# InnaBoby/Speech-Enhancement-via-Hybrid-Vision-Transformer-Project

Measured on AMD Instinct MI355X. Metric: spectrogram-frames/sec/GPU (fwd+bwd) on 256x256 mag-spec, batch 32; 1/2/4/8 GPU, higher is better.
Workload: dtype bf16; 1 GPU; HybridViT default (enc 64/128/256, 6x8-head d512 ViT, dec 256/128/64/1) train step: fwd + CombinedLoss + bwd + clip + AdamW; global_batch=32, seq_len=256, parallelism=dp1

## Files before the change

include/hvit.h:

```cpp
#ifndef HVIT_H_
#define HVIT_H_

#ifdef __cplusplus
extern "C" {
#endif

enum { HVIT_F32 = 0, HVIT_BF16 = 1 };
enum { HVIT_OK = 0, HVIT_ERR_ARG = 1, HVIT_ERR_LAUNCH = 2 };
enum {
  HVIT_ACT_NONE = 0,
  HVIT_ACT_GELU_DUAL = 1,
  HVIT_ACT_TANH = 2,
  HVIT_ACT_GELU_BWD = 3,
  HVIT_ACT_GELU_DUAL_D = 4,
  HVIT_ACT_MUL_AUX = 5,
  HVIT_ACT_RELU = 6,
  HVIT_ACT_GELU = 7,
  HVIT_ACT_RELU_POOL2 = 8,
  HVIT_ACT_GELU_DUAL_DK = 9
};
enum { HVIT_ACC_ZEROED = 1,
       HVIT_ACC_DEFER = 2 };

typedef struct {
// ... 25 lines not shown
  int rowadd_rows;
  float* colsum;
  hvit_slab_sum_t side;
} hvit_epilogue_t;

typedef struct {
  const void* src1;
  int C1;
  const void* src2;
  int C2;
  int N, Hs, Ws, U;
  int KS, stride, pad;
  int Cout;
} hvit_conv_geom_t;

const char* hvit_last_error(void);
const char* hvit_version(void);

int hvit_linear_fwd(int dt, const void* x, const void* w, const float* bias, int M, int N, int K, void* y,
                    int y_dt, const hvit_epilogue_t* epi, void* stream);
int hvit_linear_dgrad(int dt, const void* dy, const void* w, int M, int N, int K, void* dx, int dx_dt,
                      const hvit_epilogue_t* epi, void* stream);
long long hvit_wgrad_workspace(int M, int N, int K);
long long hvit_wgrad_tickets(int M, int N, int K);
int hvit_linear_wgrad_tk(int dt, const void* dy, const void* x, int M, int N, int K, float* dw, float* db, float* ws,
                         long long ws_elems, unsigned* tickets, long long tickets_elems, int flags, void* stream);
enum {
  HVIT_TUNE_RING = 0,
  HVIT_TUNE_C1_MFMA = 1,
  HVIT_TUNE_ATTN_BWD = 4,
  HVIT_TUNE_FP8_FWD = 5,
  HVIT_TUNE_WGRAD_GROUP = 7,
  HVIT_TUNE_CONV_HALO = 9,
  HVIT_TUNE_CONV_HALO_COUNT = 10
};
int hvit_gemm_tune(int what, int value);
int hvit_conv_halo_off(int H, int W, int C, int rows, int hy, int hx, int chunk);
int hvit_linear_wgrad(int dt, const void* dy, const void* x, int M, int N, int K, float* dw, float* db,
                      float* ws, long long ws_elems, void* stream);
int hvit_linear_wgrad_defer(int dt, const void* dy, const void* x, int M, int N, int K, float* dw, float* ws,
                            long long ws_elems, const hvit_slab_sum_t* side, hvit_slab_sum_t* job, void* stream);
int hvit_linear_wgrad_bias_defer(int dt, const void* dy, const void* x, int M, int N, int K, float* dw, float* db,
                                 float* ws, long long ws_elems, const hvit_slab_sum_t* side, hvit_slab_sum_t* job,
                                 void* stream);
int hvit_sum_slabs_strided(const float* ws, int splits, long long stride, long long n, float* out, void* stream);

typedef struct {
  const void* dy;
  int ldy;
  const void* x;
  int ldx;
  float* dw;
  int n_out, k_in;
  int patch, img_h, img_w, img_c;
} hvit_wgrad_prob_t;
int hvit_linear_wgrad_group_ok(int dt, int M, int n_out, int k_in);
int hvit_linear_wgrad_group_patch_ok(int dt, int M, int n_out, int patch, int img_h, int img_w, int img_c);
long long hvit_linear_wgrad_group_ws(void);
long long hvit_linear_wgrad_group_tickets(void);
int hvit_linear_wgrad_group(int dt, int M, const hvit_wgrad_prob_t* probs, int nprobs, float* ws, long long ws_elems,
                            unsigned* tickets, long long n_tickets, void* stream);

int hvit_conv_bn_tile_rows(const hvit_conv_geom_t* g);
int hvit_conv_fwd(int dt, const hvit_conv_geom_t* g, const void* w_packed, const float* bias, void* y, int y_dt,
                  float* bn_partials, const hvit_epilogue_t* epi, void* stream);
int hvit_conv_dgrad(int dt, const hvit_conv_geom_t* g, const void* dy, const void* w_packed, void* dx, int dx_dt,
                    void* stream);
long long hvit_conv_wgrad_workspace(const hvit_conv_geom_t* g);
int hvit_conv_wgrad(int dt, const hvit_conv_geom_t* g, const void* dy, float* dw_packed, float* ws,
                    long long ws_elems, void* stream);
int hvit_conv_wgrad_torch(int dt, const hvit_conv_geom_t* g, const void* dy, float* dw, float* dw_packed, float* ws,
                          long long ws_elems, void* stream);
int hvit_conv_weight_pack(const float* w, int Cout, int Cin, int KS, int mode, void* out, int out_dt,
                          void* stream);
int hvit_conv_weight_unpack(const float* dw_packed, int Cout, int Cin, int KS, float* dw, void* stream);
int hvit_bn_fold(const float* w, int Cout, int Cin, int KS, const float* mean, const float* invstd,
                 const float* gamma, const float* beta, void* w_packed, int w_dt, float* bias, void* stream);

int hvit_mhsa_fwd(int dt, const void* qkv, int B, int N, int H, int hd, float scale,
                  const hvit_dropout_t* dropout, void* o, float* lse, float* probs, void* stream);
int hvit_mhsa_bwd(int dt, const void* qkv, const void* o, const void* dout, const float* lse, int B, int N, int H,
                  int hd, float scale, const hvit_dropout_t* dropout, void* dqkv, float* delta_ws, void* stream);
long long hvit_mhsa_keep_bits_elems(int B, int N, int H);
int hvit_mhsa_keep_bits_used(int dt, int N, int hd);
int hvit_mhsa_fwd_kb(int dt, const void* qkv, int B, int N, int H, int hd, float scale, const hvit_dropout_t* dropout,
                     void* o, float* lse, unsigned* keep_bits, void* stream);
int hvit_mhsa_bwd_kb(int dt, const void* qkv, const void* o, const void* dout, const float* lse, int B, int N, int H,
                     int hd, float scale, const hvit_dropout_t* dropout, const unsigned* keep_bits, void* dqkv,
                     float* delta_ws, void* stream);
long long hvit_mhsa_bias_rows(int dt, int B, int N, int H, int hd);
int hvit_mhsa_bwd_db(int dt, const void* qkv, const void* o, const void* dout, const float* lse, int B, int N, int H,
                     int hd, float scale, const hvit_dropout_t* dropout, const unsigned* keep_bits, void* dqkv,
                     float* delta_ws, float* dbias_rows, void* stream);
int hvit_mhsa_fwd_fp8(const void* qkv, int B, int N, int H, int hd, float scale, const hvit_dropout_t* dropout,
                      void* o, float* lse, void* stream);
int hvit_mhsa_fwd_fp8_kb(const void* qkv, int B, int N, int H, int hd, float scale, const hvit_dropout_t* dropout,
                         void* o, float* lse, unsigned* keep_bits, void* stream);

int hvit_layernorm_fwd(const float* x, const float* gamma, const float* beta, int M, int D, float eps, void* y,
                       int y_dt, float* mean, float* rstd, void* stream);
long long hvit_layernorm_bwd_ws_elems(int M, int D);
long long hvit_layernorm_bwd_drop_ws_elems(int M, int D);
int hvit_layernorm_bwd_drop(const void* dy, int dy_dt, const float* x, const float* mean, const float* rstd,
                            const float* gamma, int M, int D, const float* resid, float* dx, float* acc3,
                            const hvit_dropout_t* dropout, const float* rowscale, int rows_per_sample, void* g_out,
                            int g_dt, float* ws, long long ws_elems, int flags, void* stream);
int hvit_layernorm_bwd(const void* dy, int dy_dt, const float* x, const float* mean, const float* rstd,
                       const float* gamma, int M, int D, const float* resid, float* dx, float* dgamma,
                       float* dbeta, float* ws, long long ws_elems, int flags, void* stream);

long long hvit_bn_act_bwd_sums_elems(int C);
int hvit_bn_finalize(float* partials, int ntiles, int tile_rows, long long M, int C, float* mean,
                     float* invstd, float* running_mean, float* running_var, long long* num_batches_tracked,
                     float momentum, float eps, void* stream);
int hvit_bn_eval_prep(const float* running_mean, const float* running_var, int C, float eps, float* mean,
                      float* invstd, void* stream);
int hvit_bn_act_fwd(int dt, const void* z, int N, int H, int W, int C, const float* mean, const float* invstd,
                    const float* gamma, const float* beta, const hvit_dropout_t* dropout2d, int pool, void* y,
                    int y_dt, void* stream);
int hvit_bn_act_bwd(int dt, const void* z, int N, int H, int W, int C, const float* mean, const float* invstd,
                    const float* gamma, const float* beta, const hvit_dropout_t* dropout2d, int pool,
                    const void* dy, int dy_dt, int training, void* dz, int dz_dt, float* sums, int flags,
                    void* stream);

int hvit_c1block_stats(int dt, const hvit_conv_geom_t* g, const void* w_packed, float* bn_partials, void* stream);
int hvit_c1block_fwd(int dt, const hvit_conv_geom_t* g, const void* w_packed, const float* mean,
// ... 107 lines not shown
```

speech-enhancement-via-hybrid-vision-transformer-project_amd/_lib.py:

```python

from __future__ import annotations

import ctypes as C
import os
import threading

import torch

F32, BF16 = 0, 1
ACT_NONE, ACT_GELU_DUAL, ACT_TANH, ACT_GELU_BWD, ACT_GELU_DUAL_D, ACT_MUL_AUX, ACT_RELU, ACT_GELU, ACT_RELU_POOL2 = (
    0, 1, 2, 3, 4, 5, 6, 7, 8)
ACT_GELU_DUAL_DK = 9
ACC_ZEROED = 1
ACC_DEFER = 2
TUNE_RING, TUNE_C1_MFMA, TUNE_ATTN_BWD, TUNE_FP8_FWD, TUNE_WGRAD_GROUP, TUNE_CONV_HALO, TUNE_CONV_HALO_COUNT = (
    0, 1, 4, 5, 7, 9, 10)

_HERE = os.path.dirname(os.path.abspath(__file__))
LIB_PATH = os.path.join(_HERE, os.environ.get("HVIT_LIB", "libhvit.so"))

vp = C.c_void_p
i32 = C.c_int
i64 = C.c_longlong
f32 = C.c_float
f64 = C.c_double


class Dropout(C.Structure):
    _fields_ = [("p", C.c_float), ("seed", C.c_ulonglong), ("site", C.c_uint), ("seed_ptr", C.c_void_p)]


class SlabSum(C.Structure):
    _fields_ = [("src", vp), ("dst", vp), ("n", i64), ("stride", i64), ("splits", i32)]


class WgradProb(C.Structure):
    _fields_ = [("dy", vp), ("ldy", i32), ("x", vp), ("ldx", i32), ("dw", vp), ("n_out", i32), ("k_in", i32),
                ("patch", i32), ("img_h", i32), ("img_w", i32), ("img_c", i32)]


class Epilogue(C.Structure):
    _fields_ = [
        ("act", i32), ("out2", vp), ("out2_dt", i32), ("aux", vp), ("aux_dt", i32),
        ("dropout", Dropout), ("resid", vp), ("rowscale", vp), ("rows_per_sample", i32),
        ("rowadd", vp), ("rowadd_rows", i32), ("colsum", vp), ("side", SlabSum),
    ]


class ConvGeom(C.Structure):
# ... 40 lines not shown
    "hvit_last_error": ([], C.c_char_p),
    "hvit_version": ([], C.c_char_p),
    "hvit_linear_fwd": ([i32, vp, vp, vp, i32, i32, i32, vp, i32, P(Epilogue), vp], i32),
    "hvit_linear_dgrad": ([i32, vp, vp, i32, i32, i32, vp, i32, P(Epilogue), vp], i32),
    "hvit_wgrad_workspace": ([i32, i32, i32], i64),
    "hvit_linear_wgrad": ([i32, vp, vp, i32, i32, i32, vp, vp, vp, i64, vp], i32),
    "hvit_wgrad_tickets": ([i32, i32, i32], i64),
    "hvit_linear_wgrad_defer": ([i32, vp, vp, i32, i32, i32, vp, vp, i64, P(SlabSum), P(SlabSum), vp], i32),
    "hvit_linear_wgrad_bias_defer": ([i32, vp, vp, i32, i32, i32, vp, vp, vp, i64, P(SlabSum), P(SlabSum), vp],
                                     i32),
    "hvit_mhsa_bias_rows": ([i32, i32, i32, i32, i32], i64),
    "hvit_sum_slabs_strided": ([vp, i32, i64, i64, vp, vp], i32),
    "hvit_linear_wgrad_group_ok": ([i32, i32, i32, i32], i32),
    "hvit_linear_wgrad_group_patch_ok": ([i32, i32, i32, i32, i32, i32, i32], i32),
    "hvit_linear_wgrad_group_ws": ([], i64),
    "hvit_linear_wgrad_group_tickets": ([], i64),
    "hvit_linear_wgrad_group": ([i32, i32, P(WgradProb), i32, vp, i64, vp, i64, vp], i32),
    "hvit_linear_wgrad_tk": ([i32, vp, vp, i32, i32, i32, vp, vp, vp, i64, vp, i64, i32, vp], i32),
    "hvit_conv_fwd": ([i32, P(ConvGeom), vp, vp, vp, i32, vp, P(Epilogue), vp], i32),
    "hvit_conv_dgrad": ([i32, P(ConvGeom), vp, vp, vp, i32, vp], i32),
    "hvit_conv_wgrad_workspace": ([P(ConvGeom)], i64),
    "hvit_conv_wgrad": ([i32, P(ConvGeom), vp, vp, vp, i64, vp], i32),
    "hvit_conv_wgrad_torch": ([i32, P(ConvGeom), vp, vp, vp, vp, i64, vp], i32),
    "hvit_conv_weight_pack": ([vp, i32, i32, i32, i32, vp, i32, vp], i32),
    "hvit_conv_weight_unpack": ([vp, i32, i32, i32, vp, vp], i32),
    "hvit_bn_fold": ([vp, i32, i32, i32, vp, vp, vp, vp, vp, i32, vp, vp], i32),
    "hvit_mhsa_fwd": ([i32, vp, i32, i32, i32, i32, f32, P(Dropout), vp, vp, vp, vp], i32),
    "hvit_mhsa_fwd_fp8": ([vp, i32, i32, i32, i32, f32, P(Dropout), vp, vp, vp], i32),
    "hvit_mhsa_fwd_fp8_kb": ([vp, i32, i32, i32, i32, f32, P(Dropout), vp, vp, vp, vp], i32),
    "hvit_mhsa_bwd": ([i32, vp, vp, vp, vp, i32, i32, i32, i32, f32, P(Dropout), vp, vp, vp], i32),
    "hvit_mhsa_keep_bits_elems": ([i32, i32, i32], i64),
    "hvit_mhsa_keep_bits_used": ([i32, i32, i32], i32),
    "hvit_mhsa_fwd_kb": ([i32, vp, i32, i32, i32, i32, f32, P(Dropout), vp, vp, vp, vp], i32),
    "hvit_mhsa_bwd_kb": ([i32, vp, vp, vp, vp, i32, i32, i32, i32, f32, P(Dropout), vp, vp, vp, vp], i32),
    "hvit_mhsa_bwd_db": ([i32, vp, vp, vp, vp, i32, i32, i32, i32, f32, P(Dropout), vp, vp, vp, vp, vp], i32),
    "hvit_layernorm_fwd": ([vp, vp, vp, i32, i32, f32, vp, i32, vp, vp, vp], i32),
    "hvit_layernorm_bwd_ws_elems": ([i32, i32], i64),
    "hvit_layernorm_bwd_drop_ws_elems": ([i32, i32], i64),
    "hvit_layernorm_bwd_drop": ([vp, i32, vp, vp, vp, vp, i32, i32, vp, vp, vp, P(Dropout), vp, i32, vp, i32, vp,
                                 i64, i32, vp], i32),
    "hvit_layernorm_bwd": ([vp, i32, vp, vp, vp, vp, i32, i32, vp, vp, vp, vp, vp, i64, i32, vp], i32),
    "hvit_bn_finalize": ([vp, i32, i32, i64, i32, vp, vp, vp, vp, vp, f32, f32, vp], i32),
    "hvit_bn_eval_prep": ([vp, vp, i32, f32, vp, vp, vp], i32),
    "hvit_bn_act_fwd": ([i32, vp, i32, i32, i32, i32, vp, vp, vp, vp, P(Dropout), i32, vp, i32, vp], i32),
    "hvit_bn_act_bwd": ([i32, vp, i32, i32, i32, i32, vp, vp, vp, vp, P(Dropout), i32, vp, i32, i32, vp,
                         i32, vp, i32, vp], i32),
    "hvit_bn_act_bwd_sums_elems": ([i32], i64),
    "hvit_c1block_stats": ([i32, P(ConvGeom), vp, vp, vp], i32),
    "hvit_c1block_fwd": ([i32, P(ConvGeom), vp, vp, vp, vp, vp, P(Dropout), i32, vp, i32, vp], i32),
    "hvit_c1block_bwd_ws": ([P(ConvGeom), i32], i64),
    "hvit_c1block_bwd": ([i32, P(ConvGeom), vp, vp, vp, vp, vp, P(Dropout), i32, vp, i32, i32, vp, i32, vp, vp,
                          i64, vp], i32),
    "hvit_bilinear_fwd":([vp, i32, i32, i32, i32, i32, i32, i32, vp, i32, vp], i32),
    "hvit_bilinear_bwd": ([vp, i32, i32, i32, i32, i32, i32, i32, vp, i32, i32, vp], i32),
    "hvit_upsample_split_bwd": ([vp, i32, i32, i32, i32, i32, i32, i32, vp, i32, vp, i32, vp], i32),
    "hvit_cast": ([vp, i32, vp, i32, i64, vp], i32),
    "hvit_dropout_scale": ([vp, i32, i64, i32, P(Dropout), vp, i32, vp, i32, vp, vp, i64, vp], i32),
    "hvit_dropout_colsum_ws_elems": ([i32], i64),
    "hvit_tanh_bwd": ([vp, i32, vp, i64, vp, i32, vp], i32),
    "hvit_reduce_rows": ([vp, i32, i64, i64, i64, i32, vp, vp], i32),
    "hvit_sum_slabs": ([vp, i32, i64, vp, vp], i32),
    "hvit_droppath_scale": ([i32, P(Dropout), vp, vp], i32),
    "hvit_droppath_scales": ([i32, i32, P(Dropout), vp, vp], i32),
    "hvit_weight_prep": ([i32, P(WPrepItem), vp], i32),
    "hvit_conv_bn_tile_rows": ([P(ConvGeom)], i32),
    "hvit_loss_ws_elems": ([i32, i64], i64),
# ... 102 lines not shown
```

speech-enhancement-via-hybrid-vision-transformer-project_amd/csrc/attention.hip:

```cpp
#include <algorithm>
#include <cstdlib>

#include "attention_tile.h"
#include "common.h"

namespace hvit {

constexpr int AT_THREADS = 256;
constexpr int AT_TILE = 64;

template <typename T>
__device__ __forceinline__ f32x4 mma_step(u32x4 a, u32x4 b, f32x4 c) {
  if constexpr (sizeof(T) == 2) {
    return __builtin_amdgcn_mfma_f32_16x16x32_bf16(__builtin_bit_cast(s16x8, a),
                                                   __builtin_bit_cast(s16x8, b), c, 0, 0, 0);
  } else {
    f32x4 va = __builtin_bit_cast(f32x4, a), vb = __builtin_bit_cast(f32x4, b);
    c = __builtin_amdgcn_mfma_f32_16x16x4f32(va[0], vb[0], c, 0, 0, 0);
    c = __builtin_amdgcn_mfma_f32_16x16x4f32(va[1], vb[1], c, 0, 0, 0);
    c = __builtin_amdgcn_mfma_f32_16x16x4f32(va[2], vb[2], c, 0, 0, 0);
    c = __builtin_amdgcn_mfma_f32_16x16x4f32(va[3], vb[3], c, 0, 0, 0);
    return c;
  }
}
// ... 387 lines not shown
#pragma unroll
      for (int r = 0; r < 4; ++r)
        *(T*)(Pw + (4 * fq + r) * GK::PITCH + (16 * j + frow) * sizeof(T)) = Elem<T>::from_f(s[j][r]);
    lds_fence();
#pragma unroll
    for (int st = 0; st < GK::STEPS; ++st) {
      u32x4 pa = frag<GK>(Pw, frow, st, fq);
#pragma unroll
      for (int t = 0; t < NT; ++t) dk[t] = mma_step<T>(pa, frag<GK>(Qt, 16 * t + frow, st, fq), dk[t]);
    }
    lds_fence();
  }
#pragma unroll
  for (int r = 0; r < 4; ++r) {
    int kj = key0 + 4 * fq + r;
    if (kj >= N) continue;
    T* row = dqkv + ((long)b * N + kj) * pitch + h * HD;
#pragma unroll
    for (int t = 0; t < NT; ++t) {
      row[D + 16 * t + frow] = Elem<T>::from_f(dk[t][r] * scale);
      row[2 * D + 16 * t + frow] = Elem<T>::from_f(dv[t][r]);
    }
  }
}

constexpr int V2_KMAX = 512;

template <int WAVES, int KMAX, bool FULL = false>
__global__ __launch_bounds__(WAVES * 64) void mhsa_fwd_v2(const bf16_t* __restrict__ qkv, bf16_t* __restrict__ o,
                                                         float* __restrict__ lse, int N, int H, float scale,
                                                         uint32_t thr, float dscale, DSeed seed_,
                                                         uint32_t site, uint32_t* __restrict__ kbits) {
  const unsigned long long seed = seed_;
  constexpr int CH = 256;
  __shared__ __attribute__((aligned(16))) char smem[2 * KMAX * V2_ROWB];
  char* Ks = smem;
  char* Vs = smem + KMAX * V2_ROWB;
  const int D = H * 64;
  const long pitch = 3L * D;
  const int h = blockIdx.y, b = blockIdx.z;
  const int lane = threadIdx.x & 63, w = threadIdx.x >> 6;
  const int frow = lane & 15, fq = lane >> 4;
  const V2Lane LN(lane);
  const bf16_t* base = qkv + (long)b * N * pitch + h * 64;
  const int NK32 = (N + 31) & ~31;
  const int q = blockIdx.x * WAVES * 16 + w * 16 + frow;
  const bool qin = FULL || q < N;
  u32x4 qf[2];
#pragma unroll
  for (int s2 = 0; s2 < 2; ++s2)
    qf[s2] = qin ? *(const u32x4*)(base + (long)q * pitch + 32 * s2 + 8 * fq) : (u32x4){0u, 0u, 0u, 0u};
  v2_stage_glds<WAVES>(Ks, base + D, pitch, N, NK32);
  v2_stage_glds<WAVES>(Vs, base + 2 * D, pitch, N, NK32);
  __syncthreads();
  const float c2 = scale * 1.4426950408889634f;
  const uint64_t bh = (uint64_t)b * H + h;
  const uint64_t BHN = (uint64_t)gridDim.z * H * N;
  const uint32_t rk = rng_key(seed, site);
  const uint64_t qrow = (bh * N + (qin ? q : 0)) * (uint64_t)N;
  const uint32_t hq = (uint32_t)(qrow >> 1) + 2u * (uint32_t)fq;
  f32x4 ot[4];
#pragma unroll
  for (int t = 0; t < 4; ++t) ot[t] = (f32x4){0.f, 0.f, 0.f, 0.f};
  float mxc = -INFINITY, sum = 0.f;
  auto chunk = [&](auto c0c) {
    constexpr int c0 = decltype(c0c)::value;
    const int nkt = FULL ? CH / 16 : (min(N - c0, CH) + 15) >> 4;
    const char* Kc = Ks + c0 * V2_ROWB;
    const char* Vc = Vs + c0 * V2_ROWB;
    f32x4 st[CH / 16];
    float mx = -INFINITY;
#pragma unroll
    for (int j = 0; j < CH / 16; ++j) {
      if (j < nkt) {
        f32x4 a = {0.f, 0.f, 0.f, 0.f};
        a = v2_mma32(v2_fragj(Kc, LN, j, 0), qf[0], a);
        a = v2_mma32(v2_fragj(Kc, LN, j, 1), qf[1], a);
        v2_settle(a);
        if (!FULL && c0 + 16 * j + 16 > N) {
#pragma unroll
          for (int r = 0; r < 4; ++r)
            if (c0 + 16 * j + 4 * fq + r >= N) a[r] = -INFINITY;
        }
#pragma unroll
        for (int r = 0; r < 4; ++r) mx = fmaxf(mx, a[r]);
        st[j] = a;
      }
    }
    mx = fmaxf(mx, __shfl_xor(mx, 16, 64));
    mx = fmaxf(mx, __shfl_xor(mx, 32, 64));
    const float mnew = fmaxf(mxc, mx * c2);
    if constexpr (c0 > 0) {
      const float rs = __builtin_amdgcn_exp2f(mxc - mnew);
      sum *= rs;
#pragma unroll
      for (int t = 0; t < 4; ++t) ot[t] *= rs;
    }
    mxc = mnew;
    float csum = 0.f;
#pragma unroll
    for (int j = 0; j < CH / 16; ++j) {
      if (j < nkt) {
#pragma unroll
        for (int r = 0; r < 4; ++r) {
          const float pv = __builtin_amdgcn_exp2f(fmaf(st[j][r], c2, -mxc));
          st[j][r] = pv;
          csum += pv;
        }
      }
    }
    csum += __shfl_xor(csum, 16, 64);
    csum += __shfl_xor(csum, 32, 64);
    sum += csum;
    uint32_t kb[2] = {0u, 0u};
#pragma unroll
    for (int jp = 0; jp < CH / 32; ++jp) {
      if (2 * jp < nkt) {
        f32x4 p0 = st[2 * jp];
        f32x4 p1 = (2 * jp + 1 < nkt) ? st[2 * jp + 1] : (f32x4){0.f, 0.f, 0.f, 0.f};
        if (thr) {
          uint32_t b8 = 0u;
#pragma unroll
          for (int e = 0; e < 2; ++e) {
            const int j = 2 * jp + e;
            if (j < nkt) {
              const uint32_t nib = v2_keep_step(rk, hq + (uint32_t)(c0 / 2 + 8 * j), thr, e ? p1 : p0);
              b8 |= nib << (kb_nibble(j) - kb_nibble(2 * jp));
            }
          }
          kb[kb_nibble(2 * jp) >> 5] |= b8 << (kb_nibble(2 * jp) & 31);
        }
        const u32x4 pb = v2_cat(v2_pack(p0), v2_pack(p1));
#pragma unroll
        for (int t = 0; t < 4; ++t) ot[t] = v2_mma32(v2_trj2(Vc, LN, 2 * jp, t), pb, ot[t]);
      }
    }
    if (qin && kbits && thr)
      *(uint2*)(kbits + kb_pair(c0 / CH, BHN, bh * N, q, fq)) = make_uint2(kb[0], kb[1]);
  };
  chunk(std::integral_constant<int, 0>());
  if constexpr (KMAX > CH) {
    if (N > CH) chunk(std::integral_constant<int, CH>());
  }
  if (qin) {
    const float inv = 1.f / sum;
    const float os = thr ? inv * dscale : inv;
    v2_store_row(o + ((long)b * N + q) * D + h * 64, ot, os, fq);
    if (fq == 0) lse[bh * N + q] = (mxc + log2f(sum)) * 0.6931471805599453f;
  }
}

template <int WAVES, int KMAX>
__global__ __launch_bounds__(WAVES * 64) void mhsa_dq_v2(const bf16_t* __restrict__ qkv, const bf16_t* __restrict__ o,
                                                        const bf16_t* __restrict__ dout,
                                                        const float* __restrict__ lse, float* __restrict__ delta,
                                                        bf16_t* __restrict__ dqkv, int N, int H, float scale,
                                                        uint32_t thr, float dscale, DSeed seed_,
                                                        uint32_t site, const uint32_t* __restrict__ kbits,
                                                        float* __restrict__ dbias) {
  const unsigned long long seed = seed_;
  __shared__ __attribute__((aligned(16))) char smem[2 * KMAX * V2_ROWB + WAVES * 64 * 4];
  char* Ks = smem;
  char* Vs = smem + KMAX * V2_ROWB;
  const int D = H * 64;
  const long pitch = 3L * D;
  const int h = blockIdx.y, b = blockIdx.z;
  const int lane = threadIdx.x & 63, w = threadIdx.x >> 6;
  const int frow = lane & 15, fq = lane >> 4;
  const V2Lane LN(lane);
  const bf16_t* base = qkv + (long)b * N * pitch + h * 64;
  const int NK = (N + 15) & ~15;
  const int nkt = NK >> 4;
  const int q = blockIdx.x * WAVES * 16 + w * 16 + frow;
  const bool qv = q < N;
  const uint64_t bh = (uint64_t)b * H + h;
  u32x4 qf[2], df[2];
  float dl = 0.f;
#pragma unroll
  for (int s2 = 0; s2 < 2; ++s2) {
    qf[s2] = df[s2] = (u32x4){0u, 0u, 0u, 0u};
    if (qv) {
      qf[s2] = *(const u32x4*)(base + (long)q * pitch + 32 * s2 + 8 * fq);
// ... 651 lines not shown
```

speech-enhancement-via-hybrid-vision-transformer-project_amd/csrc/attention_tile.h:

```cpp
#pragma once
#include "common.h"

namespace hvit {

constexpr int V2_ROWB = 128;
typedef short v4s_t __attribute__((ext_vector_type(4)));
typedef __attribute__((address_space(3))) v4s_t lds_v4s_t;

__device__ __forceinline__ int v2_off(int row, int chunk) { return row * V2_ROWB + ((chunk ^ (row & 7)) << 4); }

template <int WAVES>
__device__ __forceinline__ void v2_stage_glds(char* dst, const bf16_t* src, long pitch, int n, int rows) {
  const int lane = threadIdx.x & 63, w = threadIdx.x >> 6;
  const int rl = lane >> 3, cp = lane & 7;
  for (int pc = w; pc < (rows >> 3); pc += WAVES) {
    const int row = pc * 8 + rl;
    const int srow = row < n ? row : n - 1;
    const bf16_t* g = src + (long)srow * pitch + ((cp ^ rl) << 3);
    __builtin_amdgcn_global_load_lds((const __attribute__((address_space(1))) void*)g,
                                     (__attribute__((address_space(3))) void*)(dst + pc * 1024), 16, 0, 0);
  }
}
__device__ __forceinline__ u32x4 v2_frag(const char* img, int row, int s, int fq) {
  return *(const u32x4*)(img + v2_off(row, 4 * s + fq));
}
__device__ __forceinline__ v4s_t v2_tr(const char* img, int k0, int c0, int lane) {
  const int g = lane >> 4, li = lane & 15;
  const int row = k0 + 4 * g + (li >> 2);
  const int col = c0 + 4 * (li & 3);
  const char* a = img + row * V2_ROWB + (((col >> 3) ^ (row & 7)) << 4) + (col & 7) * 2;
  return __builtin_amdgcn_ds_read_tr16_b64_v4i16((lds_v4s_t*)a);
}
struct V2Lane {
// ... 110 lines not shown
#pragma unroll
  for (int r = 0; r < 4; ++r) {
    float kp = 1.f;
    if constexpr (MODE == V2_KEEP_BITS) {
      kp = ((kw4[r] >> kshift) & 1u) ? dscale : 0.f;
    }
    if constexpr (MODE == V2_KEEP_NONE) {
      pd[r] = p[r];
      ds[r] = p[r] * (dp[r] - d4[r]);
    } else {
      pd[r] = p[r] * kp;
      ds[r] = p[r] * fmaf(dp[r], kp, -d4[r]);
    }
  }
}

__device__ __forceinline__ float v2_dot8(float acc, const u32x4& x, const u32x4& y) {
#pragma unroll
  for (int e = 0; e < 4; ++e)
    acc += __uint_as_float(x[e] << 16) * __uint_as_float(y[e] << 16) +
           __uint_as_float(x[e] & 0xffff0000u) * __uint_as_float(y[e] & 0xffff0000u);
  return acc;
}
__device__ __forceinline__ void v2_store_row(bf16_t* row, const f32x4 (&acc)[4], float mul, int fq) {
#pragma unroll
  for (int t = 0; t < 4; ++t) {
    uint2 u;
    u.x = f2bf2(acc[t][0] * mul, acc[t][1] * mul);
    u.y = f2bf2(acc[t][2] * mul, acc[t][3] * mul);
    *(uint2*)(row + 16 * t + 4 * fq) = u;
  }
}

}
```

speech-enhancement-via-hybrid-vision-transformer-project_amd/csrc/capi.cpp:

```cpp
#include <stdarg.h>
#include <stdio.h>

#include "../../include/hvit.h"

static thread_local char g_err[1024] = "";

void hvit_set_error(const char* fmt, ...) {
  va_list ap;
  va_start(ap, fmt);
  vsnprintf(g_err, sizeof(g_err), fmt, ap);
  va_end(ap);
}

extern "C" const char* hvit_last_error(void) { return g_err; }

extern "C" const char* hvit_version(void) { return "hvit 0.1 gfx950"; }

int hvit_ring_tune(int value);
int hvit_c1_tune(int value);
int hvit_attn_tune(int value);
int hvit_fp8_tune(int value);
int hvit_wgrad_group_tune(int value);
int hvit_conv_halo_tune(int value);
int hvit_conv_halo_count();

extern "C" int hvit_gemm_tune(int what, int value) {
  switch (what) {
    case HVIT_TUNE_RING: return hvit_ring_tune(value);
    case HVIT_TUNE_C1_MFMA: return hvit_c1_tune(value);
    case HVIT_TUNE_ATTN_BWD: return hvit_attn_tune(value);
    case HVIT_TUNE_FP8_FWD: return hvit_fp8_tune(value);
    case HVIT_TUNE_WGRAD_GROUP: return hvit_wgrad_group_tune(value);
    case HVIT_TUNE_CONV_HALO: return hvit_conv_halo_tune(value);
    case HVIT_TUNE_CONV_HALO_COUNT: return hvit_conv_halo_count();
    default: return -1;
  }
}
```

speech-enhancement-via-hybrid-vision-transformer-project_amd/functional.py:

```python

from __future__ import annotations

import math
import os
from dataclasses import dataclass, field
from typing import Optional

import ctypes as C
import weakref

import torch

from . import _lib as L
from ._lib import call, ptr, stream_ptr

F32, BF16 = L.F32, L.BF16


OP_TIMES = None


_DEPTH = 0


# ... 33 lines not shown

    def __exit__(self, *exc):
        return False


_UNTIMED = _Untimed()


def timed(name: str, work: float):
    return _UNTIMED if OP_TIMES is None else _Timed(name, work)


REPLAY = None


def _record(name, fn):
    if REPLAY is not None:
        REPLAY.setdefault(name, []).append(fn)


def _launch(name, work, fn, e=None, keep=()):
    with timed(name, work):
        fn(e)
    if REPLAY is not None:
        er = None
        if e is not None:
            er = type(e).from_buffer_copy(e)
            er.side = L.SlabSum()
        _record(name, ((lambda er=er, keep=keep: fn(er, stream_ptr())), work))


def _empty(shape, dt, dev):
    return torch.empty(shape, dtype=L.torch_dtype(dt), device=dev)


class ZSlot:

    __slots__ = ("n", "t", "__weakref__")

    def __init__(self, n):
        self.n = n
        self.t = None

    def take(self, dev):
        t, self.t = self.t, None
        return t if t is not None else torch.zeros(self.n, dtype=torch.float32, device=dev)


_ZPENDING = []


def zslot(n: int) -> ZSlot:
    s = ZSlot(n)
    if len(_ZPENDING) > 4096:
        _ZPENDING[:] = [r for r in _ZPENDING if r() is not None]
    _ZPENDING.append(weakref.ref(s))
    return s


def zflush(dev) -> None:
    live = [s for s in (r() for r in _ZPENDING) if s is not None and s.t is None]
    _ZPENDING.clear()
    if not live:
        return
    offs, tot = [], 0
    for s in live:
# ... 882 lines not shown
    if not sites:
        return
    out = torch.empty((len(sites), 2 * B), dtype=torch.float32, device=dev)
    for k in range(0, len(sites), 32):
        part = sites[k:k + 32]
        arr = (L.Dropout * len(part))()
        keep = []
        for i, (p, d) in enumerate(part):
            arr[i] = L.dropout(p, d.seed, 1, d.seed_t)
            keep.append(arr[i])
        call("hvit_droppath_scales", 2 * B, len(part), arr, out[k].data_ptr(), stream_ptr())
    for i, (_, d) in enumerate(sites):
        d.pre = out[i]


class ViTBlockFn(torch.autograd.Function):

    @staticmethod
    def forward(ctx, x, n1w, n1b, qkvw, qkvb, pw, pb, n2w, n2b, f1w, f1b, f2w, f2b, H, drops, dpr, training,
                dt, want_probs, attn_fp8=False, ho_in: Optional[GradHandoff] = None,
                ho_out: Optional[GradHandoff] = None, nograd: bool = False):
        B, Nt, D = x.shape
        M = B * Nt
        hd = D // H
        hid = f1w.shape[0]
        dev = x.device
        s = stream_ptr()
        scale = hd ** -0.5
        x2d = x.contiguous().view(M, D)
        d_attn, d_proj, d_fc1, d_fc2, dp_seed = drops if training else (Drop(),) * 4 + (0,)
        rs1, rs2 = droppath_scales(B, dpr if training else 0.0, dp_seed, dev)
        xn1, m1, r1 = _ln(x2d, n1w, n1b, dt)
        Wqkv = cast(qkvw, dt)
        qkv = _empty((M, 3 * D), dt, dev)
        _launch("vit_linear_fwd", 2.0 * M * 3 * D * D,
                lambda e, st=s: call("hvit_linear_fwd", dt, xn1.data_ptr(), Wqkv.data_ptr(), qkvb.data_ptr(), M, 3 * D, D,
                               qkv.data_ptr(), dt, e, st))
        o = _empty((M, D), dt, dev)
        lse = torch.empty((B, H, Nt), dtype=torch.float32, device=dev)
        kbits = None
        probs = torch.empty((B, H, Nt, Nt), dtype=torch.float32, device=dev) if want_probs else None
        if attn_fp8 and not want_probs:
            if dt != BF16:
                raise ValueError("hvit: the fp8 attention path runs inside the bf16 model (precision='bf16')")
            if d_attn.p > 0 and KEEPBITS and L.lib().hvit_mhsa_keep_bits_used(dt, Nt, hd):
                kbits = torch.empty(L.lib().hvit_mhsa_keep_bits_elems(B, Nt, H), dtype=torch.int32, device=dev)
            with timed("attn_fwd", 4.0 * B * H * Nt * Nt * hd):
                call("hvit_mhsa_fwd_fp8_kb", qkv.data_ptr(), B, Nt, H, hd, scale, d_attn.c(), o.data_ptr(),
                     lse.data_ptr(), ptr(kbits), s)
        elif probs is None and d_attn.p > 0 and KEEPBITS and L.lib().hvit_mhsa_keep_bits_used(dt, Nt, hd):
            kbits = torch.empty(L.lib().hvit_mhsa_keep_bits_elems(B, Nt, H), dtype=torch.int32, device=dev)
            with timed("attn_fwd", 4.0 * B * H * Nt * Nt * hd):
                call("hvit_mhsa_fwd_kb", dt, qkv.data_ptr(), B, Nt, H, hd, scale, d_attn.c(), o.data_ptr(),
                     lse.data_ptr(), kbits.data_ptr(), s)
        else:
            with timed("attn_fwd", 4.0 * B * H * Nt * Nt * hd):
                call("hvit_mhsa_fwd", dt, qkv.data_ptr(), B, Nt, H, hd, scale, d_attn.c(), o.data_ptr(),
                     lse.data_ptr(), ptr(probs), s)
        Wp = cast(pw, dt)
        x1 = torch.empty((M, D), dtype=torch.float32, device=dev)
        _launch("vit_linear_fwd", 2.0 * M * D * D,
                lambda e, st=s: call("hvit_linear_fwd", dt, o.data_ptr(), Wp.data_ptr(), pb.data_ptr(), M, D, D,
                               x1.data_ptr(), F32, e, st),
                epilogue(drop=d_proj.c(), resid=x2d, rowscale=rs1, rps=Nt), (x2d, rs1))
        xn2, m2, r2 = _ln(x1, n2w, n2b, dt)
        W1 = cast(f1w, dt)
        a = _empty((M, hid), dt, dev)
        if not nograd:
            gh = _empty((M, hid), dt, dev)
            _launch("vit_linear_fwd", 2.0 * M * hid * D,
                    lambda e, st=s: call("hvit_linear_fwd", dt, xn2.data_ptr(), W1.data_ptr(), f1b.data_ptr(), M, hid, D,
                                   gh.data_ptr(), dt, e, st),
                    epilogue(act=L.ACT_GELU_DUAL_DK, out2=a, drop=d_fc1.c()), (a,))
        else:
            gh = None
# ... 265 lines not shown
```

Measured before the change: 1.898 million spectrogram-frames/s.

## Fuse QKV projection GEMM with flash attention forward per batch-head block

```diff
diff --git a/include/hvit.h b/include/hvit.h
--- a/include/hvit.h
+++ b/include/hvit.h
@@ -81,7 +81,8 @@
   HVIT_TUNE_FP8_FWD = 5,
   HVIT_TUNE_WGRAD_GROUP = 7,
   HVIT_TUNE_CONV_HALO = 9,
-  HVIT_TUNE_CONV_HALO_COUNT = 10
+  HVIT_TUNE_CONV_HALO_COUNT = 10,
+  HVIT_TUNE_QKV_ATTN_FUSED = 11
 };
 int hvit_gemm_tune(int what, int value);
 int hvit_conv_halo_off(int H, int W, int C, int rows, int hy, int hx, int chunk);
@@ -141,6 +142,10 @@
 int hvit_mhsa_bwd_db(int dt, const void* qkv, const void* o, const void* dout, const float* lse, int B, int N, int H,
                      int hd, float scale, const hvit_dropout_t* dropout, const unsigned* keep_bits, void* dqkv,
                      float* delta_ws, float* dbias_rows, void* stream);
+int hvit_qkv_mhsa_fused_used(int dt, int N, int hd, int D);
+int hvit_qkv_mhsa_fwd(int dt, const void* x, const void* w, const float* bias, int B, int N, int H, int hd,
+                      float scale, const hvit_dropout_t* dropout, void* qkv, void* o, float* lse, unsigned* keep_bits,
+                      void* stream);
 int hvit_mhsa_fwd_fp8(const void* qkv, int B, int N, int H, int hd, float scale, const hvit_dropout_t* dropout,
                       void* o, float* lse, void* stream);
 int hvit_mhsa_fwd_fp8_kb(const void* qkv, int B, int N, int H, int hd, float scale, const hvit_dropout_t* dropout,
diff --git a/speech-enhancement-via-hybrid-vision-transformer-project_amd/_lib.py b/speech-enhancement-via-hybrid-vision-transformer-project_amd/_lib.py
--- a/speech-enhancement-via-hybrid-vision-transformer-project_amd/_lib.py
+++ b/speech-enhancement-via-hybrid-vision-transformer-project_amd/_lib.py
@@ -15,6 +15,7 @@
 ACC_DEFER = 2
 TUNE_RING, TUNE_C1_MFMA, TUNE_ATTN_BWD, TUNE_FP8_FWD, TUNE_WGRAD_GROUP, TUNE_CONV_HALO, TUNE_CONV_HALO_COUNT = (
     0, 1, 4, 5, 7, 9, 10)
+TUNE_QKV_ATTN_FUSED = 11
 
 _HERE = os.path.dirname(os.path.abspath(__file__))
 LIB_PATH = os.path.join(_HERE, os.environ.get("HVIT_LIB", "libhvit.so"))
@@ -121,6 +122,8 @@
     "hvit_mhsa_keep_bits_elems": ([i32, i32, i32], i64),
     "hvit_mhsa_keep_bits_used": ([i32, i32, i32], i32),
     "hvit_mhsa_fwd_kb": ([i32, vp, i32, i32, i32, i32, f32, P(Dropout), vp, vp, vp, vp], i32),
+    "hvit_qkv_mhsa_fused_used": ([i32, i32, i32, i32], i32),
+    "hvit_qkv_mhsa_fwd": ([i32, vp, vp, vp, i32, i32, i32, i32, f32, P(Dropout), vp, vp, vp, vp, vp], i32),
     "hvit_mhsa_bwd_kb": ([i32, vp, vp, vp, vp, i32, i32, i32, i32, f32, P(Dropout), vp, vp, vp, vp], i32),
     "hvit_mhsa_bwd_db": ([i32, vp, vp, vp, vp, i32, i32, i32, i32, f32, P(Dropout), vp, vp, vp, vp, vp], i32),
     "hvit_layernorm_fwd": ([vp, vp, vp, i32, i32, f32, vp, i32, vp, vp, vp], i32),
diff --git a/speech-enhancement-via-hybrid-vision-transformer-project_amd/csrc/attention.hip b/speech-enhancement-via-hybrid-vision-transformer-project_amd/csrc/attention.hip
--- a/speech-enhancement-via-hybrid-vision-transformer-project_amd/csrc/attention.hip
+++ b/speech-enhancement-via-hybrid-vision-transformer-project_amd/csrc/attention.hip
@@ -443,7 +443,6 @@
                                                          uint32_t thr, float dscale, DSeed seed_,
                                                          uint32_t site, uint32_t* __restrict__ kbits) {
   const unsigned long long seed = seed_;
-  constexpr int CH = 256;
   __shared__ __attribute__((aligned(16))) char smem[2 * KMAX * V2_ROWB];
   char* Ks = smem;
   char* Vs = smem + KMAX * V2_ROWB;
@@ -464,101 +463,8 @@
   v2_stage_glds<WAVES>(Ks, base + D, pitch, N, NK32);
   v2_stage_glds<WAVES>(Vs, base + 2 * D, pitch, N, NK32);
   __syncthreads();
-  const float c2 = scale * 1.4426950408889634f;
-  const uint64_t bh = (uint64_t)b * H + h;
-  const uint64_t BHN = (uint64_t)gridDim.z * H * N;
-  const uint32_t rk = rng_key(seed, site);
-  const uint64_t qrow = (bh * N + (qin ? q : 0)) * (uint64_t)N;
-  const uint32_t hq = (uint32_t)(qrow >> 1) + 2u * (uint32_t)fq;
-  f32x4 ot[4];
-#pragma unroll
-  for (int t = 0; t < 4; ++t) ot[t] = (f32x4){0.f, 0.f, 0.f, 0.f};
-  float mxc = -INFINITY, sum = 0.f;
-  auto chunk = [&](auto c0c) {
-    constexpr int c0 = decltype(c0c)::value;
-    const int nkt = FULL ? CH / 16 : (min(N - c0, CH) + 15) >> 4;
-    const char* Kc = Ks + c0 * V2_ROWB;
-    const char* Vc = Vs + c0 * V2_ROWB;
-    f32x4 st[CH / 16];
-    float mx = -INFINITY;
-#pragma unroll
-    for (int j = 0; j < CH / 16; ++j) {
-      if (j < nkt) {
-        f32x4 a = {0.f, 0.f, 0.f, 0.f};
-        a = v2_mma32(v2_fragj(Kc, LN, j, 0), qf[0], a);
-        a = v2_mma32(v2_fragj(Kc, LN, j, 1), qf[1], a);
-        v2_settle(a);
-        if (!FULL && c0 + 16 * j + 16 > N) {
-#pragma unroll
-          for (int r = 0; r < 4; ++r)
-            if (c0 + 16 * j + 4 * fq + r >= N) a[r] = -INFINITY;
-        }
-#pragma unroll
-        for (int r = 0; r < 4; ++r) mx = fmaxf(mx, a[r]);
-        st[j] = a;
-      }
-    }
-    mx = fmaxf(mx, __shfl_xor(mx, 16, 64));
-    mx = fmaxf(mx, __shfl_xor(mx, 32, 64));
-    const float mnew = fmaxf(mxc, mx * c2);
-    if constexpr (c0 > 0) {
-      const float rs = __builtin_amdgcn_exp2f(mxc - mnew);
-      sum *= rs;
-#pragma unroll
-      for (int t = 0; t < 4; ++t) ot[t] *= rs;
-    }
-    mxc = mnew;
-    float csum = 0.f;
-#pragma unroll
-    for (int j = 0; j < CH / 16; ++j) {
-      if (j < nkt) {
-#pragma unroll
-        for (int r = 0; r < 4; ++r) {
-          const float pv = __builtin_amdgcn_exp2f(fmaf(st[j][r], c2, -mxc));
-          st[j][r] = pv;
-          csum += pv;
-        }
-      }
-    }
-    csum += __shfl_xor(csum, 16, 64);
-    csum += __shfl_xor(csum, 32, 64);
-    sum += csum;
-    uint32_t kb[2] = {0u, 0u};
-#pragma unroll
-    for (int jp = 0; jp < CH / 32; ++jp) {
-      if (2 * jp < nkt) {
-        f32x4 p0 = st[2 * jp];
-        f32x4 p1 = (2 * jp + 1 < nkt) ? st[2 * jp + 1] : (f32x4){0.f, 0.f, 0.f, 0.f};
-        if (thr) {
-          uint32_t b8 = 0u;
-#pragma unroll
-          for (int e = 0; e < 2; ++e) {
-            const int j = 2 * jp + e;
-            if (j < nkt) {
-              const uint32_t nib = v2_keep_step(rk, hq + (uint32_t)(c0 / 2 + 8 * j), thr, e ? p1 : p0);
-              b8 |= nib << (kb_nibble(j) - kb_nibble(2 * jp));
-            }
-          }
-          kb[kb_nibble(2 * jp) >> 5] |= b8 << (kb_nibble(2 * jp) & 31);
-        }
-        const u32x4 pb = v2_cat(v2_pack(p0), v2_pack(p1));
-#pragma unroll
-        for (int t = 0; t < 4; ++t) ot[t] = v2_mma32(v2_trj2(Vc, LN, 2 * jp, t), pb, ot[t]);
-      }
-    }
-    if (qin && kbits && thr)
-      *(uint2*)(kbits + kb_pair(c0 / CH, BHN, bh * N, q, fq)) = make_uint2(kb[0], kb[1]);
-  };
-  chunk(std::integral_constant<int, 0>());
-  if constexpr (KMAX > CH) {
-    if (N > CH) chunk(std::integral_constant<int, CH>());
-  }
-  if (qin) {
-    const float inv = 1.f / sum;
-    const float os = thr ? inv * dscale : inv;
-    v2_store_row(o + ((long)b * N + q) * D + h * 64, ot, os, fq);
-    if (fq == 0) lse[bh * N + q] = (mxc + log2f(sum)) * 0.6931471805599453f;
-  }
+  v2_fwd_body<KMAX, FULL>(Ks, Vs, LN, qf, frow, fq, q, b, h, (uint32_t)gridDim.z, o, lse, N, H, scale, thr, dscale, seed,
+                          site, kbits);
 }
 
 template <int WAVES, int KMAX>
diff --git a/speech-enhancement-via-hybrid-vision-transformer-project_amd/csrc/attention_tile.h b/speech-enhancement-via-hybrid-vision-transformer-project_amd/csrc/attention_tile.h
--- a/speech-enhancement-via-hybrid-vision-transformer-project_amd/csrc/attention_tile.h
+++ b/speech-enhancement-via-hybrid-vision-transformer-project_amd/csrc/attention_tile.h
@@ -1,4 +1,6 @@
 #pragma once
+#include <type_traits>
+
 #include "common.h"
 
 namespace hvit {
@@ -175,4 +177,112 @@
   }
 }
 
-}
+template <int KMAX, bool FULL>
+__device__ __forceinline__ void v2_fwd_body(char* const& Ks, char* const& Vs, const V2Lane& LN,
+                                            const u32x4 (&qf)[2], const int& frow, const int& fq, const int& q,
+                                            const int& b, const int& h, const uint32_t& B,
+                                            bf16_t* __restrict__ const& o, float* __restrict__ const& lse,
+                                            const int& N, const int& H, const float& scale, const uint32_t& thr,
+                                            const float& dscale, const unsigned long long& seed,
+                                            const uint32_t& site, uint32_t* __restrict__ const& kbits) {
+  constexpr int CH = 256;
+  const int D = H * 64;
+  const bool qin = FULL || q < N;
+  const float c2 = scale * 1.4426950408889634f;
+  const uint64_t bh = (uint64_t)b * H + h;
+  const uint64_t BHN = (uint64_t)B * H * N;
+  const uint32_t rk = rng_key(seed, site);
+  const uint64_t qrow = (bh * N + (qin ? q : 0)) * (uint64_t)N;
+  const uint32_t hq = (uint32_t)(qrow >> 1) + 2u * (uint32_t)fq;
+  f32x4 ot[4];
+#pragma unroll
+  for (int t = 0; t < 4; ++t) ot[t] = (f32x4){0.f, 0.f, 0.f, 0.f};
+  float mxc = -INFINITY, sum = 0.f;
+  auto chunk = [&](auto c0c) {
+    constexpr int c0 = decltype(c0c)::value;
+    const int nkt = FULL ? CH / 16 : (min(N - c0, CH) + 15) >> 4;
+    const char* Kc = Ks + c0 * V2_ROWB;
+    const char* Vc = Vs + c0 * V2_ROWB;
+    f32x4 st[CH / 16];
+    float mx = -INFINITY;
+#pragma unroll
+    for (int j = 0; j < CH / 16; ++j) {
+      if (j < nkt) {
+        f32x4 a = {0.f, 0.f, 0.f, 0.f};
+        a = v2_mma32(v2_fragj(Kc, LN, j, 0), qf[0], a);
+        a = v2_mma32(v2_fragj(Kc, LN, j, 1), qf[1], a);
+        v2_settle(a);
+        if (!FULL && c0 + 16 * j + 16 > N) {
+#pragma unroll
+          for (int r = 0; r < 4; ++r)
+            if (c0 + 16 * j + 4 * fq + r >= N) a[r] = -INFINITY;
+        }
+#pragma unroll
+        for (int r = 0; r < 4; ++r) mx = fmaxf(mx, a[r]);
+        st[j] = a;
+      }
+    }
+    mx = fmaxf(mx, __shfl_xor(mx, 16, 64));
+    mx = fmaxf(mx, __shfl_xor(mx, 32, 64));
+    const float mnew = fmaxf(mxc, mx * c2);
+    if constexpr (c0 > 0) {
+      const float rs = __builtin_amdgcn_exp2f(mxc - mnew);
+      sum *= rs;
+#pragma unroll
+      for (int t = 0; t < 4; ++t) ot[t] *= rs;
+    }
+    mxc = mnew;
+    float csum = 0.f;
+#pragma unroll
+    for (int j = 0; j < CH / 16; ++j) {
+      if (j < nkt) {
+#pragma unroll
+        for (int r = 0; r < 4; ++r) {
+          const float pv = __builtin_amdgcn_exp2f(fmaf(st[j][r], c2, -mxc));
+          st[j][r] = pv;
+          csum += pv;
+        }
+      }
+    }
+    csum += __shfl_xor(csum, 16, 64);
+    csum += __shfl_xor(csum, 32, 64);
+    sum += csum;
+    uint32_t kb[2] = {0u, 0u};
+#pragma unroll
+    for (int jp = 0; jp < CH / 32; ++jp) {
+      if (2 * jp < nkt) {
+        f32x4 p0 = st[2 * jp];
+        f32x4 p1 = (2 * jp + 1 < nkt) ? st[2 * jp + 1] : (f32x4){0.f, 0.f, 0.f, 0.f};
+        if (thr) {
+          uint32_t b8 = 0u;
+#pragma unroll
+          for (int e = 0; e < 2; ++e) {
+            const int j = 2 * jp + e;
+            if (j < nkt) {
+              const uint32_t nib = v2_keep_step(rk, hq + (uint32_t)(c0 / 2 + 8 * j), thr, e ? p1 : p0);
+              b8 |= nib << (kb_nibble(j) - kb_nibble(2 * jp));
+            }
+          }
+          kb[kb_nibble(2 * jp) >> 5] |= b8 << (kb_nibble(2 * jp) & 31);
+        }
+        const u32x4 pb = v2_cat(v2_pack(p0), v2_pack(p1));
+#pragma unroll
+        for (int t = 0; t < 4; ++t) ot[t] = v2_mma32(v2_trj2(Vc, LN, 2 * jp, t), pb, ot[t]);
+      }
+    }
+    if (qin && kbits && thr)
+      *(uint2*)(kbits + kb_pair(c0 / CH, BHN, bh * N, q, fq)) = make_uint2(kb[0], kb[1]);
+  };
+  chunk(std::integral_constant<int, 0>());
+  if constexpr (KMAX > CH) {
+    if (N > CH) chunk(std::integral_constant<int, CH>());
+  }
+  if (qin) {
+    const float inv = 1.f / sum;
+    const float os = thr ? inv * dscale : inv;
+    v2_store_row(o + ((long)b * N + q) * D + h * 64, ot, os, fq);
+    if (fq == 0) lse[bh * N + q] = (mxc + log2f(sum)) * 0.6931471805599453f;
+  }
+}
+
+}
diff --git a/speech-enhancement-via-hybrid-vision-transformer-project_amd/csrc/capi.cpp b/speech-enhancement-via-hybrid-vision-transformer-project_amd/csrc/capi.cpp
--- a/speech-enhancement-via-hybrid-vision-transformer-project_amd/csrc/capi.cpp
+++ b/speech-enhancement-via-hybrid-vision-transformer-project_amd/csrc/capi.cpp
@@ -23,6 +23,7 @@
 int hvit_wgrad_group_tune(int value);
 int hvit_conv_halo_tune(int value);
 int hvit_conv_halo_count();
+int hvit_qkv_attn_tune(int value);
 
 extern "C" int hvit_gemm_tune(int what, int value) {
   switch (what) {
@@ -33,6 +34,7 @@
     case HVIT_TUNE_WGRAD_GROUP: return hvit_wgrad_group_tune(value);
     case HVIT_TUNE_CONV_HALO: return hvit_conv_halo_tune(value);
     case HVIT_TUNE_CONV_HALO_COUNT: return hvit_conv_halo_count();
+    case HVIT_TUNE_QKV_ATTN_FUSED: return hvit_qkv_attn_tune(value);
     default: return -1;
   }
 }
diff --git a/speech-enhancement-via-hybrid-vision-transformer-project_amd/csrc/qkv_attention.hip b/speech-enhancement-via-hybrid-vision-transformer-project_amd/csrc/qkv_attention.hip
--- /dev/null
+++ b/speech-enhancement-via-hybrid-vision-transformer-project_amd/csrc/qkv_attention.hip
@@ -0,0 +1,184 @@
+#include "attention_tile.h"
+#include "common.h"
+#include "gemm_ring.h"
+
+namespace hvit {
+
+constexpr int QA_N = 256;
+using QaImgX = DmaImg<QA_N, true>;
+using QaImgW = DmaImg<64, true>;
+constexpr int QA_WBYTES = 3 * QaImgW::BYTES;
+constexpr int QA_STAGE = QA_WBYTES + QaImgX::BYTES;
+constexpr int QA_IMG = QA_N * V2_ROWB;
+constexpr int QA_SMEM = 2 * QA_STAGE > 3 * QA_IMG ? 2 * QA_STAGE : 3 * QA_IMG;
+static_assert(QaImgX::PIECES == 32 && QaImgW::PIECES == 8, "pieces per stage");
+
+template <int OFF>
+__device__ __forceinline__ u32x4 ds128_asm(unsigned addr) {
+  u32x4 r;
+  asm volatile("ds_read_b128 %0, %1 offset:%2" : "=v"(r) : "v"(addr), "n"(OFF));
+  return r;
+}
+
+__global__ __launch_bounds__(1024) void qkv_mhsa_fwd_fused(const bf16_t* __restrict__ x, const bf16_t* __restrict__ wq,
+                                                           const float* __restrict__ bias, bf16_t* __restrict__ qkv,
+                                                           bf16_t* __restrict__ o, float* __restrict__ lse, int H,
+                                                           float scale, uint32_t thr, float dscale, DSeed seed_,
+                                                           uint32_t site, uint32_t* __restrict__ kbits) {
+  const unsigned long long seed = seed_;
+  __shared__ __attribute__((aligned(1024))) char smem[QA_SMEM];
+  const int D = H * 64;
+  const TileId bh3 = tile_of(1);
+  const int b = bh3.mt, h = bh3.nt;
+  const uint32_t B = gridDim.x;
+  const int tid = threadIdx.x, lane = tid & 63;
+  const int wid = __builtin_amdgcn_readfirstlane(tid >> 6);
+  const int frow = lane & 15, fq = lane >> 4;
+  const int wn = wid & 3, wm = wid >> 2;
+  const int nk = D / 64;
+
+  const bf16_t* xb = x + (long)b * QA_N * D;
+  const bf16_t* wh = wq + (long)h * 64 * D;
+  const __amdgpu_buffer_rsrc_t rx = __builtin_amdgcn_make_buffer_rsrc((void*)xb, (short)0, QA_N * D * 2, 0x00020000);
+  const __amdgpu_buffer_rsrc_t rw =
+      __builtin_amdgcn_make_buffer_rsrc((void*)wh, (short)0, (2 * D + 64) * D * 2, 0x00020000);
+  const unsigned vx0 = QaImgX::src_off(wid, lane, D), vx1 = QaImgX::src_off(wid + 16, lane, D);
+  const unsigned sbytes = (unsigned)D * (unsigned)D * 2u;
+  const unsigned vw0 = QaImgW::src_off(wid & 7, lane, D) + (unsigned)(wid >> 3) * sbytes;
+  const unsigned vw1 = QaImgW::src_off(wid & 7, lane, D) + 2u * sbytes;
+  auto issue = [&](int t) {
+    char* wbuf = smem + (t & 1) * QA_STAGE;
+    char* xbuf = wbuf + QA_WBYTES;
+    const unsigned so = (unsigned)t * 128u;
+    __builtin_amdgcn_raw_ptr_buffer_load_lds(rx, (__attribute__((address_space(3))) void*)(xbuf + wid * 1024), 16, vx0,
+                                             so, 0, 0);
+    __builtin_amdgcn_raw_ptr_buffer_load_lds(rx, (__attribute__((address_space(3))) void*)(xbuf + (wid + 16) * 1024),
+                                             16, vx1, so, 0, 0);
+    __builtin_amdgcn_raw_ptr_buffer_load_lds(rw, (__attribute__((address_space(3))) void*)(wbuf + wid * 1024), 16, vw0,
+                                             so, 0, 0);
+    if (wid < 8)
+      __builtin_amdgcn_raw_ptr_buffer_load_lds(rw, (__attribute__((address_space(3))) void*)(wbuf + (wid + 16) * 1024),
+                                               16, vw1, so, 0, 0);
+  };
+  const unsigned lds0 = lds_addr(smem);
+  unsigned aw[2], ax[2];
+#pragma unroll
+  for (int s = 0; s < 2; ++s) {
+    aw[s] = lds0 + kc_off(48 * wn + frow, 4 * s + fq);
+    ax[s] = lds0 + QA_WBYTES + kc_off(64 * wm + frow, 4 * s + fq);
+  }
+  f32x4 acc[3][4];
+#pragma unroll
+  for (int i = 0; i < 3; ++i)
+#pragma unroll
+    for (int j = 0; j < 4; ++j) acc[i][j] = (f32x4){0.f, 0.f, 0.f, 0.f};
+  f32x4 bv[3];
+#pragma unroll
+  for (int i = 0; i < 3; ++i) {
+    const int n = 48 * wn + 16 * i + 4 * fq;
+    bv[i] = bias ? *(const f32x4*)(bias + (n >> 6) * D + h * 64 + (n & 63)) : (f32x4){0.f, 0.f, 0.f, 0.f};
+  }
+
+  issue(0);
+  for (int t = 0; t < nk; ++t) {
+    __builtin_amdgcn_s_waitcnt(vm_imm(0));
+    asm volatile("" ::: "memory");
+    __builtin_amdgcn_s_barrier();
+    asm volatile("" ::: "memory");
+    const unsigned bo = (unsigned)(t & 1) * QA_STAGE;
+#pragma unroll
+    for (int s = 0; s < 2; ++s) {
+      u32x4 fw[3], fx[4];
+      const unsigned a = aw[s] + bo, c = ax[s] + bo;
+      fw[0] = ds128_asm<0>(a);
+      fw[1] = ds128_asm<2048>(a);
+      fw[2] = ds128_asm<4096>(a);
+      fx[0] = ds128_asm<0>(c);
+      fx[1] = ds128_asm<2048>(c);
+      fx[2] = ds128_asm<4096>(c);
+      fx[3] = ds128_asm<6144>(c);
+      if (s == 0 && t + 1 < nk) issue(t + 1);
+      lgkm_wait0();
+      lds_pin(fw);
+      lds_pin(fx);
+#pragma unroll
+      for (int i = 0; i < 3; ++i)
+#pragma unroll
+        for (int j = 0; j < 4; ++j)
+          acc[i][j] = __builtin_amdgcn_mfma_f32_16x16x32_bf16(__builtin_bit_cast(s16x8, fw[i]),
+                                                              __builtin_bit_cast(s16x8, fx[j]), acc[i][j], 0, 0, 0);
+    }
+  }
+  __syncthreads();
+
+#pragma unroll
+  for (int i = 0; i < 3; ++i) {
+    const int n0 = 48 * wn + 16 * i;
+    char* img = smem + (n0 >> 6) * QA_IMG;
+    const int d0 = (n0 & 63) + 4 * fq;
+#pragma unroll
+    for (int j = 0; j < 4; ++j) {
+      const f32x4 v = acc[i][j] + bv[i];
+      uint2 u;
+      u.x = f2bf2(v[0], v[1]);
+      u.y = f2bf2(v[2], v[3]);
+      *(uint2*)(img + v2_off(64 * wm + 16 * j + frow, d0 >> 3) + (d0 & 7) * 2) = u;
+    }
+  }
+  __syncthreads();
+  if (qkv) {
+#pragma unroll
+    for (int u = 0; u < 3 * QA_IMG / 16 / 1024; ++u) {
+      const int c = tid + 1024 * u;
+      const int strip = c >> 11, row = (c >> 3) & (QA_N - 1), ch = c & 7;
+      const u32x4 v = *(const u32x4*)(smem + strip * QA_IMG + v2_off(row, ch));
+      bf16_t* dst = qkv + ((long)b * QA_N + row) * (3L * D) + strip * D + h * 64 + ch * 8;
+      __builtin_nontemporal_store(v, (u32x4*)dst);
+    }
+  }
+  const V2Lane LN(lane);
+  const int w = tid >> 6;
+  u32x4 qf[2];
+#pragma unroll
+  for (int s2 = 0; s2 < 2; ++s2) qf[s2] = v2_fragj(smem, LN, w, s2);
+
+  v2_fwd_body<QA_N, true>(smem + QA_IMG, smem + 2 * QA_IMG, LN, qf, frow, fq, 16 * w + frow, b, h, B, o, lse, QA_N, H,
+                          scale, thr, dscale, seed, site, kbits);
+}
+
+static int& qkv_attn_ref() {
+  static int v = 1;
+  return v;
+}
+
+}
+
+using namespace hvit;
+
+int hvit_qkv_attn_tune(int value) {
+  const int old = qkv_attn_ref();
+  if (value == 0 || value == 1) qkv_attn_ref() = value;
+  return old;
+}
+
+extern "C" int hvit_qkv_mhsa_fused_used(int dt, int N, int hd, int D) {
+  return qkv_attn_ref() != 0 && dt == HVIT_BF16 && hd == 64 && N == QA_N && D >= 64 && D % 64 == 0 ? 1 : 0;
+}
+
+extern "C" int hvit_qkv_mhsa_fwd(int dt, const void* x, const void* w, const float* bias, int B, int N, int H, int hd,
+                                 float scale, const hvit_dropout_t* dropout, void* qkv, void* o, float* lse,
+                                 unsigned* keep_bits, void* stream) {
+  HVIT_CHECK(x && w && o && lse, "hvit_qkv_mhsa_fwd: null pointer");
+  HVIT_CHECK(B > 0 && H > 0 && B <= 65535 && H <= 65535, "hvit_qkv_mhsa_fwd: bad shape B=%d H=%d", B, H);
+  HVIT_CHECK(hvit_qkv_mhsa_fused_used(dt, N, hd, H * hd),
+             "hvit_qkv_mhsa_fwd: no fused kernel for dt=%d N=%d hd=%d (hvit_qkv_mhsa_fused_used)", dt, N, hd);
+  HVIT_CHECK(aligned16(x) && aligned16(w) && aligned16(bias) && aligned16(qkv) && aligned16(o) && aligned16(keep_bits),
+             "hvit_qkv_mhsa_fwd: tensors must be 16-byte aligned");
+  HVIT_CHECK((2L * H * 64 + 64) * H * 64 * 2 < (1L << 31), "hvit_qkv_mhsa_fwd: W_qkv too large");
+  const DropArgs da = drop_args(dropout);
+  hipLaunchKernelGGL(qkv_mhsa_fwd_fused, dim3(B, H), dim3(1024), 0, (hipStream_t)stream, (const bf16_t*)x,
+                     (const bf16_t*)w, bias, (bf16_t*)qkv, (bf16_t*)o, lse, H, scale, da.thr, da.dscale, da.seed,
+                     da.site, (uint32_t*)keep_bits);
+  HVIT_LAUNCH_CHECK();
+  return HVIT_OK;
+}
diff --git a/speech-enhancement-via-hybrid-vision-transformer-project_amd/functional.py b/speech-enhancement-via-hybrid-vision-transformer-project_amd/functional.py
--- a/speech-enhancement-via-hybrid-vision-transformer-project_amd/functional.py
+++ b/speech-enhancement-via-hybrid-vision-transformer-project_amd/functional.py
@@ -89,6 +89,11 @@
 
 def _empty(shape, dt, dev):
     return torch.empty(shape, dtype=L.torch_dtype(dt), device=dev)
+
+
+def qkv_attn_fused(dt, Nt, hd, D) -> bool:
+    used = getattr(L.lib(), "hvit_qkv_mhsa_fused_used", None)
+    return used is not None and bool(used(dt, Nt, hd, D))
 
 
 class ZSlot:
@@ -1037,15 +1042,23 @@
         rs1, rs2 = droppath_scales(B, dpr if training else 0.0, dp_seed, dev)
         xn1, m1, r1 = _ln(x2d, n1w, n1b, dt)
         Wqkv = cast(qkvw, dt)
-        qkv = _empty((M, 3 * D), dt, dev)
-        _launch("vit_linear_fwd", 2.0 * M * 3 * D * D,
-                lambda e, st=s: call("hvit_linear_fwd", dt, xn1.data_ptr(), Wqkv.data_ptr(), qkvb.data_ptr(), M, 3 * D, D,
-                               qkv.data_ptr(), dt, e, st))
+        fused = not attn_fp8 and not want_probs and qkv_attn_fused(dt, Nt, hd, D)
+        qkv = None if fused and nograd else _empty((M, 3 * D), dt, dev)
+        if not fused:
+            _launch("vit_linear_fwd", 2.0 * M * 3 * D * D,
+                    lambda e, st=s: call("hvit_linear_fwd", dt, xn1.data_ptr(), Wqkv.data_ptr(), qkvb.data_ptr(), M, 3 * D,
+                                   D, qkv.data_ptr(), dt, e, st))
         o = _empty((M, D), dt, dev)
         lse = torch.empty((B, H, Nt), dtype=torch.float32, device=dev)
         kbits = None
         probs = torch.empty((B, H, Nt, Nt), dtype=torch.float32, device=dev) if want_probs else None
-        if attn_fp8 and not want_probs:
+        if fused:
+            if d_attn.p > 0 and KEEPBITS and L.lib().hvit_mhsa_keep_bits_used(dt, Nt, hd):
+                kbits = torch.empty(L.lib().hvit_mhsa_keep_bits_elems(B, Nt, H), dtype=torch.int32, device=dev)
+            _launch("qkv_attn_fwd", 2.0 * M * 3 * D * D + 4.0 * B * H * Nt * Nt * hd,
+                    lambda e, st=s: call("hvit_qkv_mhsa_fwd", dt, xn1.data_ptr(), Wqkv.data_ptr(), qkvb.data_ptr(), B, Nt,
+                                   H, hd, scale, d_attn.c(), ptr(qkv), o.data_ptr(), lse.data_ptr(), ptr(kbits), st))
+        elif attn_fp8 and not want_probs:
             if dt != BF16:
                 raise ValueError("hvit: the fp8 attention path runs inside the bf16 model (precision='bf16')")
             if d_attn.p > 0 and KEEPBITS and L.lib().hvit_mhsa_keep_bits_used(dt, Nt, hd):
```

After: 1.921 million spectrogram-frames/s, median of 6. 1.2% higher.
